# IanYeung/RealVSR

Hardware: AMD Instinct MI355X
Metric: HR frames/sec (fwd+bwd) on 5-frame 180x320 LR windows (higher is better)
Workload: dtype f32 (bf16x3 GEMM); 1 GPU; EDVR-M nf64, 5-frame 180x320 LR windows, batch 8 per GPU, x4 output, VideoSRModel.optimize_parameters: fwd + LapPyr(ssim,cb) on Y + GWLoss on CbCr + bwd + Adam step; per_gpu_batch=8, global_batch=8, parallelism=sequence-dp1, gemm=bf16x3 (3-term bf16 split on v_mfma_f32_32x32x16_bf16, f32 accumulate), lf_term=ssim (restated IQA_pytorch.SSIM, parity unpinned)

## Files before the change

### realvsr_amd/csrc/conv2_kernels.hip

```cpp
#define RVSR_DEFINE_PACK
#include "conv_plan.h"

#include "bf16x3.h"

#ifdef RVSR_ABL5
constexpr int ABL5 = RVSR_ABL5;
#else
constexpr int ABL5 = 0;
#endif

#ifdef RVSR_TIMELINE
__device__ unsigned long long rvsr_dbg[512];
extern "C" int rvsr_debug_read(unsigned long long* out) { return (int)hipMemcpyFromSymbol(out, HIP_SYMBOL(rvsr_dbg), sizeof(unsigned long long) * 512); }
#define STAMP(i) do { if (blockIdx.x == 77 && tid == 0) rvsr_dbg[(i)] = __builtin_amdgcn_s_memtime(); } while (0)
#else
#define STAMP(i) do {} while (0)
#endif

template <int MT, int MODE>
__device__ __forceinline__ void conv2_epilogue(f32x16 (&acc)[MT][2], const ConvFwdParams& p, const float* bias_s, int b,
                                               int o0, int row0, int col, int hi) {
    const float neg = p.act == 0 ? 1.f : (p.act == 1 ? 0.f : p.slope);
    const bool col_ok = col < p.Wout;
    const size_t HW = (size_t)p.Hout * p.Wout;
// ... 76 lines not shown
                float4 v = make_float4(r0 + bb, r1 + bb, r2 + bb, r3 + bb);
                v.x = v.x > 0.f ? v.x : v.x * neg; v.y = v.y > 0.f ? v.y : v.y * neg;
                v.z = v.z > 0.f ? v.z : v.z * neg; v.w = v.w > 0.f ? v.w : v.w * neg;
                if (MODE == 1) { v.x += resv[rg].x; v.y += resv[rg].y; v.z += resv[rg].z; v.w += resv[rg].w; }
                buf_store4(out_rs, off[rg] + (unsigned)(o0 + m * 32 + 8 * rg) * HW4, 0u, v);
            }
        }
    }
}

__device__ __forceinline__ void half_swap(float& a, float& b) {
    asm volatile("s_nop 1\n\tv_permlane32_swap_b32 %0, %1\n\ts_nop 0" : "+v"(a), "+v"(b));
}
template <int MT, int MODE>
__device__ __forceinline__ void conv2_epilogue_wide(f32x16 (&acc)[MT][2], const ConvFwdParams& p, const float* bias_s, int b,
                                                    int o0, int row, int x0, int lo, int hi) {
    if (row >= p.Hout) return;
    const float neg = (p.act == 0 || MODE == 4) ? 1.f : (p.act == 1 ? 0.f : p.slope);
    const int lane = 32 * hi + lo, jn = lane >> 4, Gn = lane & 15;
    const int src4 = 4 * (4 * Gn + jn);
    const int col4 = x0 + 4 * Gn;
    const bool col_ok = col4 < p.Wout;
    const unsigned HW = (unsigned)(p.Hout * p.Wout), HW4 = 4u * HW;
    const __amdgpu_buffer_rsrc_t out_rs = buf_view_2g(p.out1 + (size_t)b * p.Co * HW);
    const __amdgpu_buffer_rsrc_t res_rs = buf_view_2g(MODE == 5   ? p.res + (size_t)(b % p.res_period) * p.Co * HW
                                                      : MODE == 1 || MODE == 4 ? p.res + (size_t)b * p.Co * HW
                                                                               : p.out1);
    const unsigned lane_off = 4u * ((unsigned)jn * HW + (unsigned)row * p.Wout + col4);
    const int j = lo & 3;
#pragma unroll
    for (int m = 0; m < MT; ++m) {
#pragma unroll
        for (int rg = 0; rg < 4; ++rg) {
            float4 resv[2];
            unsigned off[2];
#pragma unroll
            for (int s = 0; s < 2; ++s) {
                const int ob = o0 + m * 32 + 8 * rg + 4 * s;
                off[s] = col_ok && ob + jn < p.Co ? lane_off : 0x80000000u;
                if (MODE == 1 || MODE == 4 || MODE == 5) {
                    typedef float f32x4v __attribute__((ext_vector_type(4)));
                    const f32x4v q = __builtin_bit_cast(f32x4v, __builtin_amdgcn_raw_buffer_load_b128(res_rs, (int)(off[s] + (unsigned)ob * HW4), 0, 0));
                    resv[s] = make_float4(q.x, q.y, q.z, q.w);
                }
            }
            float r[2][4];
            const float bb = bias_s[m * 32 + 8 * rg + 4 * hi + j];
#pragma unroll
            for (int n = 0; n < 2; ++n) {
                r[n][0] = acc[m][n][4 * rg + 0]; r[n][1] = acc[m][n][4 * rg + 1]; r[n][2] = acc[m][n][4 * rg + 2]; r[n][3] = acc[m][n][4 * rg + 3];
                quad_transpose4(r[n][0], r[n][1], r[n][2], r[n][3], lo);
#pragma unroll
                for (int e = 0; e < 4; ++e) {
                    const float v = r[n][e] + bb;
                    r[n][e] = MODE == 5 ? v : (v > 0.f ? v : v * neg);
                }
            }
#pragma unroll
            for (int e = 0; e < 4; ++e) half_swap(r[0][e], r[1][e]);
#pragma unroll
            for (int s = 0; s < 2; ++s)
#pragma unroll
                for (int e = 0; e < 4; ++e)
                    r[s][e] = __builtin_bit_cast(float, __builtin_amdgcn_ds_bpermute(src4, __builtin_bit_cast(int, r[s][e])));
#pragma unroll
            for (int s = 0; s < 2; ++s) {
                float4 v = make_float4(r[s][0], r[s][1], r[s][2], r[s][3]);
                if (MODE == 1 || MODE == 5) { v.x += resv[s].x; v.y += resv[s].y; v.z += resv[s].z; v.w += resv[s].w; }
                if (MODE == 5) {
                    v.x = v.x > 0.f ? v.x : v.x * neg; v.y = v.y > 0.f ? v.y : v.y * neg;
                    v.z = v.z > 0.f ? v.z : v.z * neg; v.w = v.w > 0.f ? v.w : v.w * neg;
                }
                if (MODE == 4) {
                    v.x *= resv[s].x > 0.f ? 1.f : p.slope; v.y *= resv[s].y > 0.f ? 1.f : p.slope;
                    v.z *= resv[s].z > 0.f ? 1.f : p.slope; v.w *= resv[s].w > 0.f ? 1.f : p.slope;
                }
                if (!(ABL5 & 2) || (m == 0 && rg == 0 && s == 0))
                buf_store4(out_rs, off[s] + (unsigned)(o0 + m * 32 + 8 * rg + 4 * s) * HW4, 0u, v);
            }
        }
    }
}

template <int KS, int STRIDE, int MT, int CCG, bool ACT_IN, int NW>
__global__ __launch_bounds__(NW * 64, 2) void conv_fwd2_kernel(const ConvFwdParams p) {
    constexpr int T = KS * KS, PAD = KS / 2, TH = 2 * NW, TW = 32, NTHR = NW * 64;
    constexpr int IH = (TH - 1) * STRIDE + KS, IW = (TW - 1) * STRIDE + KS;
    constexpr int MP = MT * 32, NOCT = 2 * CCG, NPOS = IH * IW;
    constexpr int WVEC = T * NOCT * MP;
    extern __shared__ __attribute__((aligned(16))) unsigned char smem_raw[];
    bf16x8* xs_hi = reinterpret_cast<bf16x8*>(smem_raw);
    bf16x8* xs_lo = xs_hi + NOCT * NPOS;
    bf16x8* ws_hi = xs_lo + NOCT * NPOS;
    bf16x8* ws_lo = ws_hi + WVEC;
    float* bias_s = reinterpret_cast<float*>(ws_lo + WVEC);
    const int tid = threadIdx.x, lane = tid & 63, wave = tid >> 6, lo = lane & 31, hi = lane >> 5;
    const TView& va = p.in.a;
    const TView& vb = p.in.b;
    const int C1 = va.C, Ctot = va.C + vb.C;
    const int nchunks = (Ctot + 16 * CCG - 1) / (16 * CCG);

    const unsigned nmb = (p.Co + MP - 1) / MP, nty = (p.Hout + TH - 1) / TH, ntx = (p.Wout + TW - 1) / TW;
    const unsigned items = ntx * nty * nmb * p.B;
    const unsigned xcd = blockIdx.x & 7, wq = blockIdx.x >> 3, nwq = (gridDim.x + 7 - xcd) >> 3;
    const unsigned q8 = items >> 3, r8 = items & 7;
    const unsigned range0 = xcd < r8 ? xcd * (q8 + 1) : r8 * (q8 + 1) + (xcd - r8) * q8;
    const unsigned range1 = range0 + q8 + (xcd < r8 ? 1 : 0);

    int x0 = 0, y0 = 0, mb = 0, b = 0;
    auto decode = [&](unsigned S) {
        const unsigned t = S % (p.ntx * nty);
        x0 = (int)(t % p.ntx) * TW;
        y0 = (int)(t / p.ntx) * TH;
        mb = (int)((S / (p.ntx * nty)) % nmb);
        b = (int)(S / (p.ntx * nty * nmb));
    };

    constexpr int NIT = (NOCT * NPOS + NTHR - 1) / NTHR;
    constexpr int NWV = (2 * WVEC + NTHR - 1) / NTHR;
    float vin[NIT][8];
    float ain[ACT_IN ? NIT : 1][8];
    int nvalid[NIT];

    __amdgpu_buffer_rsrc_t xa_rs = buf_view_2g(va.p), xb_rs = buf_view_2g(va.p), act_rs = buf_view_2g(va.p);
    auto tile_views = [&]() {
        if (va.mode != 0) return;
        const size_t hw = (size_t)va.Hs * va.Ws;
        xa_rs = buf_view_2g(va.p + (size_t)b * va.C * hw);
        if (vb.C) xb_rs = buf_view_2g(vb.p + (size_t)b * vb.C * hw);
        if (ACT_IN) act_rs = buf_view_2g(va.act + (size_t)b * va.C * hw);
    };
    auto issue_loads = [&](int chunk, int i_lo = 0, int i_hi = 1 << 20) {
        const int c0 = chunk * 16 * CCG;
#pragma unroll
        for (int i = 0; i < NIT; ++i) {
            if (i < i_lo || i >= i_hi) continue;
            const int it_raw = tid + i * NTHR;
            const bool live = it_raw < NOCT * NPOS;
            const int it = live ? it_raw : 0;
            const int oc = it / NPOS, pos = it - oc * NPOS;
            const int r = pos / IW, s = pos - r * IW;
            const int gy = y0 * STRIDE - PAD + r, gx = x0 * STRIDE - PAD + s;
            const int cb = c0 + oc * 8;
            const bool inb = live && gy >= 0 && gx >= 0 && gy < va.Hv && gx < va.Wv && cb < Ctot;
            const int gyc = gy < 0 ? 0 : (gy >= va.Hv ? va.Hv - 1 : gy), gxc = gx < 0 ? 0 : (gx >= va.Wv ? va.Wv - 1 : gx);
            if (va.mode == 0) {
                const bool second = c0 >= C1;
                const int Cb = second ? vb.C : va.C, cl0 = second ? c0 - C1 : c0;
                const unsigned hw4 = 4u * (unsigned)(va.Hs * va.Ws);
                const bool pos_ok = live && gy >= 0 && gx >= 0 && gy < va.Hv && gx < va.Wv;
                const unsigned vo = pos_ok ? 4u * (unsigned)(gy * va.Ws + gx) + (unsigned)(8 * oc) * hw4 : 0x80000000u;
                const int lane_nch = Cb - cl0 - 8 * oc;
                nvalid[i] = 8;
#pragma unroll
                for (int j = 0; j < 8; ++j) {
                    const unsigned vo_j = j < lane_nch ? vo : 0x80000000u;
                    const unsigned so = (unsigned)(cl0 + j) * hw4;
                    vin[i][j] = buf_load(second ? xb_rs : xa_rs, vo_j, so);
                    if (ACT_IN) ain[i][j] = buf_load(act_rs, vo_j, so);
                }
            } else {
                const size_t hw = (size_t)va.Hs * va.Ws;
                const int cbc = inb ? cb : 0;
                const size_t base = ((size_t)b * (va.C >> 2) + (cbc >> 2)) * hw + (size_t)(2 * gyc) * va.Ws + 2 * gxc;
                nvalid[i] = inb ? 8 : 0;
#pragma unroll
                for (int j = 0; j < 8; ++j) {
                    const size_t idx = base + (j >> 2) * hw + ((j >> 1) & 1) * va.Ws + (j & 1);
                    vin[i][j] = va.p[idx];
                    if (ACT_IN) ain[i][j] = va.act[idx];
                }
            }
        }
    };
    auto commit_inputs = [&](int i_lo = 0, int i_hi = 1 << 20) {
#pragma unroll
        for (int i = 0; i < NIT; ++i) {
            if (i < i_lo || i >= i_hi) continue;
            const int it = tid + i * NTHR;
            float v[8];
#pragma unroll
            for (int j = 0; j < 8; ++j) {
                float x = ACT_IN ? vin[i][j] * (ain[i][j] > 0.f ? 1.f : va.slope) : vin[i][j];
                v[j] = j < nvalid[i] ? x : 0.f;
            }
            bf16x8 h8, l8;
            split8(v, h8, l8);
            if (it < NOCT * NPOS) {
                xs_hi[it] = h8;
                xs_lo[it] = l8;
            }
        }
    };
    auto commit_to_lds = [&](int chunk, bool inputs_done = false) {
        const bf16x8* src = reinterpret_cast<const bf16x8*>(p.wpack) + ((size_t)mb * nchunks + chunk) * 2 * WVEC;
        constexpr int WB = MT >= 4 ? 3 : 9;
        constexpr bool OVERLAP = !ACT_IN && MT <= 2;
        if (!OVERLAP && !inputs_done) commit_inputs();
#pragma unroll
        for (int base = 0; base < NWV; base += WB) {
            bf16x8 wv[WB];
#pragma unroll
            for (int i = 0; i < WB; ++i) {
                const int e = tid + (base + i) * NTHR;
                wv[i] = src[(base + i < NWV && e < 2 * WVEC) ? e : 0];
            }
            if (OVERLAP && base == 0 && !inputs_done) commit_inputs();
#pragma unroll
            for (int i = 0; i < WB; ++i) {
                const int e = tid + (base + i) * NTHR;
                if (base + i < NWV && e < 2 * WVEC) ws_hi[e] = wv[i];
            }
        }
        if (chunk == 0 && tid < MP) {
            const int o = mb * MP + tid;
            bias_s[tid] = (p.bias != nullptr && o < p.Co) ? p.bias[o] : 0.f;
        }
    };

    constexpr bool PF = !ACT_IN && MT <= 2 && STRIDE == 1;
    unsigned S = range0 + wq;
    if (S < range1) {
        decode(S);
        tile_views();
        if (PF) issue_loads(0);
    }
    for (; S < range1; S += nwq) {
        f32x16 acc[MT][2];
#pragma unroll
        for (int m = 0; m < MT; ++m) {
            acc[m][0] = zero16();
            acc[m][1] = zero16();
        }
        const int cx0 = x0, cy0 = y0, cmb = mb, cb_ = b;
        STAMP(0);
        for (int chunk = 0; chunk < nchunks; ++chunk) {
            constexpr int NB = 3;
            if (!PF && STRIDE == 2) {
#pragma unroll
                for (int i0 = 0; i0 < NIT; i0 += NB) {
                    issue_loads(chunk, i0, i0 + NB);
                    commit_inputs(i0, i0 + NB);
                }
                commit_to_lds(chunk, true);
            } else {
                if (!PF) issue_loads(chunk);
                commit_to_lds(chunk);
            }
            STAMP(1 + chunk * 5);
            __syncthreads();
            STAMP(2 + chunk * 5);
            if (PF && chunk + 1 < nchunks) issue_loads(chunk + 1);
            STAMP(3 + chunk * 5);
#pragma unroll
            for (int tap = 0; tap < T; ++tap) {
                const int dy = tap / KS, dx = tap % KS;
#pragma unroll
                for (int g = 0; g < CCG; ++g) {
                    const int oc = 2 * g + hi;
                    bf16x8 ah[MT], al[MT], bh[2], bl[2];
#pragma unroll
                    for (int m = 0; m < MT; ++m) {
                        ah[m] = ws_hi[(tap * NOCT + oc) * MP + m * 32 + lo];
                        al[m] = ws_lo[(tap * NOCT + oc) * MP + m * 32 + lo];
                    }
#pragma unroll
                    for (int n = 0; n < 2; ++n) {
                        const int idx = (oc * IH + (wave * 2 + n) * STRIDE + dy) * IW + lo * STRIDE + dx;
                        bh[n] = xs_hi[idx];
                        bl[n] = xs_lo[idx];
                    }
#pragma unroll
                    for (int m = 0; m < MT; ++m)
#pragma unroll
                        for (int n = 0; n < 2; ++n) acc[m][n] = mfma_bf16(ah[m], bh[n], acc[m][n]);
#pragma unroll
                    for (int m = 0; m < MT; ++m)
#pragma unroll
                        for (int n = 0; n < 2; ++n) acc[m][n] = mfma_bf16(ah[m], bl[n], acc[m][n]);
#pragma unroll
                    for (int m = 0; m < MT; ++m)
#pragma unroll
                        for (int n = 0; n < 2; ++n) acc[m][n] = mfma_bf16(al[m], bh[n], acc[m][n]);
                }
            }
            STAMP(4 + chunk * 5);
            __syncthreads();
            STAMP(5 + chunk * 5);
        }
        if (p.ps)
            conv2_epilogue<MT, 3>(acc, p, bias_s, cb_, cmb * MP, cy0 + wave * 2, cx0 + lo, hi);
        else if (p.out2 != nullptr)
            conv2_epilogue<MT, 2>(acc, p, bias_s, cb_, cmb * MP, cy0 + wave * 2, cx0 + lo, hi);
        else if (p.res != nullptr) {
            if (p.vec4) conv2_epilogue_v4<MT, 1>(acc, p, bias_s, cb_, cmb * MP, cy0 + wave * 2, cx0, lo, hi);
            else conv2_epilogue<MT, 1>(acc, p, bias_s, cb_, cmb * MP, cy0 + wave * 2, cx0 + lo, hi);
        } else {
            if (p.vec4) conv2_epilogue_v4<MT, 0>(acc, p, bias_s, cb_, cmb * MP, cy0 + wave * 2, cx0, lo, hi);
            else conv2_epilogue<MT, 0>(acc, p, bias_s, cb_, cmb * MP, cy0 + wave * 2, cx0 + lo, hi);
        }
        STAMP(30);
        if (S + nwq < range1) {
            decode(S + nwq);
// ... 384 lines not shown
            for (int m = 0; m < MT; ++m)
#pragma unroll
                for (int n = 0; n < 2; ++n) acc[m][n] = mfma_bf16(ah[sl][m], bh[sl][n], acc[m][n]);
            if (NT >= 2) {
#pragma unroll
                for (int m = 0; m < MT; ++m)
#pragma unroll
                    for (int n = 0; n < 2; ++n) acc[m][n] = mfma_bf16(ah[sl][m], bl[sl][n], acc[m][n]);
            }
            if (NT >= 3) {
#pragma unroll
                for (int m = 0; m < MT; ++m)
#pragma unroll
                    for (int n = 0; n < 2; ++n) acc[m][n] = mfma_bf16(al[sl][m], bh[sl][n], acc[m][n]);
            }
            }
            if (tap < 4) {
                if (pub) commit(buf ^ 1, NWV, tap);
            } else {
                if (pub) commit(buf ^ 1, tap - 4, 8);
                if (tap == 4) stage_tile(q + 2, k_nx2, c_nx2);
                issue_stage(q + 2, c_nx2, tap - 4, (ABL5 & 4) ? 8 : VEC ? (tap < 6 ? tap - 4 : 8) : (tap - 4 < NIT ? tap - 4 : 8));
            }
            __builtin_amdgcn_sched_barrier(0);
        }
        STAMP(2 + (q & 7) * 3);
#ifdef RVSR_TIMELINE
        if (blockIdx.x == 77 && lane == 0 && q == Q - 3) rvsr_dbg[70 + wave] = __builtin_amdgcn_s_memtime();
        if (blockIdx.x == 77 && lane == 0 && q == Q - 4) rvsr_dbg[90 + wave] = __builtin_amdgcn_s_memtime();
        if (blockIdx.x == 77 && lane == 0 && q == Q - 6) rvsr_dbg[300 + wave * 12 + 9] = __builtin_amdgcn_s_memtime();
#endif
        const int k = k_cur;
        const bool last_chunk = c_cur == nchunks - 1;
        if (++c_cur == nchunks) { c_cur = 0; ++k_cur; }
        if (++c_nx2 == nchunks) { c_nx2 = 0; ++k_nx2; }
        if (last_chunk) {
            const Tile cur = tile_of(k);
            const float* bias_s = bias_base + (k & 3) * MP;
            if (WIDE) {
                if (p.act == 3) conv2_epilogue_wide<MT, 4>(acc, p, bias_s, cur.b, cur.mb * MP, cur.y0 + wave, cur.x0, lo, hi);
                else if (p.res_period > 0) conv2_epilogue_wide<MT, 5>(acc, p, bias_s, cur.b, cur.mb * MP, cur.y0 + wave, cur.x0, lo, hi);
                else if (p.res != nullptr) conv2_epilogue_wide<MT, 1>(acc, p, bias_s, cur.b, cur.mb * MP, cur.y0 + wave, cur.x0, lo, hi);
                else conv2_epilogue_wide<MT, 0>(acc, p, bias_s, cur.b, cur.mb * MP, cur.y0 + wave, cur.x0, lo, hi);
            } else if (p.ps)
                conv2_epilogue<MT, 3>(acc, p, bias_s, cur.b, cur.mb * MP, cur.y0 + wave * 2, cur.x0 + lo, hi);
            else if (p.out2 != nullptr)
                conv2_epilogue<MT, 2>(acc, p, bias_s, cur.b, cur.mb * MP, cur.y0 + wave * 2, cur.x0 + lo, hi);
            else if (p.res != nullptr) {
                if (p.vec4) conv2_epilogue_v4<MT, 1>(acc, p, bias_s, cur.b, cur.mb * MP, cur.y0 + wave * 2, cur.x0, lo, hi);
                else conv2_epilogue<MT, 1>(acc, p, bias_s, cur.b, cur.mb * MP, cur.y0 + wave * 2, cur.x0 + lo, hi);
            } else {
                if (p.vec4) conv2_epilogue_v4<MT, 0>(acc, p, bias_s, cur.b, cur.mb * MP, cur.y0 + wave * 2, cur.x0, lo, hi);
                else conv2_epilogue<MT, 0>(acc, p, bias_s, cur.b, cur.mb * MP, cur.y0 + wave * 2, cur.x0 + lo, hi);
            }
#pragma unroll
            for (int m = 0; m < MT; ++m) {
                acc[m][0] = zero16();
                acc[m][1] = zero16();
            }
        }
        __syncthreads();
        STAMP(3 + (q & 7) * 3);
#ifdef RVSR_TIMELINE
        if (blockIdx.x == 77 && lane == 0 && q == Q - 4) rvsr_dbg[80 + wave] = __builtin_amdgcn_s_memtime();
        if (blockIdx.x == 77 && lane == 0 && q == Q - 6) rvsr_dbg[300 + wave * 12 + 10] = __builtin_amdgcn_s_memtime();
        if (blockIdx.x == 77 && lane == 0 && q == Q - 7) rvsr_dbg[300 + wave * 12 + 11] = __builtin_amdgcn_s_memtime();
#endif
    }
    STAMP(61);
#ifdef RVSR_TIMELINE
    if (blockIdx.x == 77 && tid == 0) rvsr_dbg[62] = (unsigned long long)Q;
#endif
}


size_t rvsr_conv_fwd2_workspace_bytes(int ksize, int Co, int Ctot) {
    int mt, ccg, nchunks, nmb;
    conv_fwd2_geom(ksize, Co, Ctot, mt, ccg, nchunks, nmb);
    return (size_t)nmb * nchunks * 2 * (ksize * ksize) * (2 * ccg) * (mt * 32) * 16;
}

typedef void (*ConvFwdKernel)(const ConvFwdParams);

static ConvFwdKernel fwd2_kernel(int ksize, int stride, const ConvFwdPlan& q) {
#define ROW(KS, STRIDE, MT, CCG) \
    if (ksize == KS && stride == STRIDE && q.mt == MT) return q.act_in ? conv_fwd2_kernel<KS, STRIDE, MT, CCG, true, 4> : conv_fwd2_kernel<KS, STRIDE, MT, CCG, false, 4>
    ROW(3, 2, 1, 1);
    ROW(3, 2, 2, 1);
    ROW(5, 1, 1, 1);
    ROW(5, 2, 1, 1);
    ROW(1, 1, 1, 2);
    ROW(1, 1, 2, 2);
#undef ROW
    return nullptr;
}

static ConvFwdKernel fwd5_kernel(const ConvFwdPlan& q) {
#define ROW(MT, VEC, WIDE, NT) \
    if (q.mt == MT && q.vec == VEC && q.wide == WIDE && q.nt == NT) return q.act_in ? conv_fwd5_kernel<MT, true, VEC, WIDE, NT> : conv_fwd5_kernel<MT, false, VEC, WIDE, NT>
    ROW(2, 1, true, 3);
    ROW(2, 1, true, 2);
    ROW(2, 1, true, 1);
    ROW(2, 1, false, 3);
    ROW(2, 1, false, 2);
    ROW(2, 1, false, 1);
    ROW(2, 2, false, 3);
    ROW(2, 2, false, 2);
    ROW(2, 2, false, 1);
    ROW(2, 3, false, 3);
    ROW(2, 3, false, 2);
    ROW(2, 3, false, 1);
    ROW(2, 0, false, 3);
    ROW(1, 0, false, 3);
    ROW(1, 1, false, 3);
    ROW(1, 2, false, 3);
    ROW(1, 3, false, 3);
#undef ROW
    if (q.mt == 2 && q.vec == 1 && q.nt == 4 && !q.act_in) return q.wide ? conv_fwd5_kernel<2, false, 1, true, 4> : conv_fwd5_kernel<2, false, 1, false, 4>;
    return nullptr;
}

int rvsr_launch_conv_fwd2(ConvFwdParams p, const ConvFwdPlan& q, int ksize, int stride, void* workspace, size_t workspace_bytes, hipStream_t st) {
    const int Ctot = p.in.a.C + p.in.b.C, T = ksize * ksize;
    int mt, ccg, nchunks, nmb;
    conv_fwd2_geom(ksize, p.Co, Ctot, mt, ccg, nchunks, nmb);
    const size_t need = rvsr_conv_fwd2_workspace_bytes(ksize, p.Co, Ctot);
    if (!workspace || workspace_bytes < need) FAIL(RVSR_ERR_WORKSPACE, "conv2d: workspace %zu B < %zu B", workspace_bytes, need);
    const bool five = q.family == CONV_FWD5;
    const ConvFwdKernel k = five ? fwd5_kernel(q) : fwd2_kernel(ksize, stride, q);
    if (!k) FAIL(RVSR_ERR_LAUNCH, "conv2d: no %s instantiation for this plan", five ? "conv_fwd5" : "conv_fwd2");
    if (!p.prepacked) {
        const size_t total = (size_t)nmb * nchunks * T * (2 * ccg) * (mt * 32);
        hipLaunchKernelGGL(pack_weights_kernel, dim3((unsigned)((total + 255) / 256)), dim3(256), 0, st, p.w, (bf16x8*)workspace, p.Co,
                           Ctot, T, mt * 32, ccg, nchunks, nmb, p.w_mode | (p.fmt ? 0x100 : 0));
    }
    p.wpack = workspace;
    p.vec4 = q.vec4;
    return rvsr_conv_launch(five ? "conv_fwd5" : "conv_fwd2", k, dim3(q.gx), five ? 512 : 256, q.lds, st, p);
}

extern "C" size_t rvsr_conv2d_pack_weights(const float* weight, int C_in, int Co, int ksize, int w_mode, void* out, size_t out_bytes,
                                           long long* desc, void* stream) {
    int mt, ccg, nchunks, nmb;
    if (ksize != 1 && ksize != 3 && ksize != 5) return 0;
    conv_fwd2_geom(ksize, Co, C_in, mt, ccg, nchunks, nmb);
    const size_t need = rvsr_conv_fwd2_workspace_bytes(ksize, Co, C_in);
    if (!weight || !out || out_bytes < need) return 0;
    if ((w_mode & 4) && !conv_f16fp8_ok(ksize, 1, mt, w_mode & 1)) return 0;
    const int fmtflag = (w_mode & 4) ? 0x100 : 0;
    const int T = ksize * ksize;
    const size_t total = (size_t)nmb * nchunks * T * (2 * ccg) * (mt * 32);
    hipLaunchKernelGGL(pack_weights_kernel, dim3((unsigned)((total + 255) / 256)), dim3(256), 0, (hipStream_t)stream, weight, (bf16x8*)out, Co,
                       C_in, T, mt * 32, ccg, nchunks, nmb, (w_mode & 1) | fmtflag);
    if (desc) {
        desc[0] = (long long)(uintptr_t)weight; desc[1] = (long long)(uintptr_t)out;
        desc[2] = Co; desc[3] = C_in; desc[4] = T; desc[5] = mt * 32; desc[6] = ccg; desc[7] = nchunks; desc[8] = nmb; desc[9] = (w_mode & 1) | fmtflag;
    }
    return need;
}
extern "C" int rvsr_pack_weights_batched(const void* descs, int n, void* stream) {
    if (n <= 0) return RVSR_OK;
    if (!descs) FAIL(RVSR_ERR_BAD_ARG, "pack_weights_batched: null table");
    static_assert(sizeof(PackDesc) == 48, "PackDesc layout is part of the C ABI (two pointers + eight ints)");
    hipLaunchKernelGGL(pack_weights_batched_kernel, dim3(16, (unsigned)n), dim3(256), 0, (hipStream_t)stream, (const PackDesc*)descs);
    hipError_t e = hipGetLastError();
    if (e != hipSuccess) FAIL(RVSR_ERR_LAUNCH, "pack_weights_batched launch: %s", hipGetErrorString(e));
    return RVSR_OK;
}

#define WG2_THREADS 512
#define WG2_GP 272
#define WG2_XP 496

typedef unsigned int u32x4 __attribute__((ext_vector_type(4)));

__device__ __forceinline__ bf16x8 as_bf16x8(u32x4 v) { return __builtin_bit_cast(bf16x8, v); }

template <int SHIFT>
__device__ __forceinline__ bf16x8 take8(u32x4 a, u32x4 b) {
    u32x4 r;
    if (SHIFT == 4) {
        r[0] = a[2]; r[1] = a[3]; r[2] = b[0]; r[3] = b[1];
    } else if (SHIFT == 3) {
        r[0] = __builtin_amdgcn_alignbit(a[2], a[1], 16);
        r[1] = __builtin_amdgcn_alignbit(a[3], a[2], 16);
        r[2] = __builtin_amdgcn_alignbit(b[0], a[3], 16);
        r[3] = __builtin_amdgcn_alignbit(b[1], b[0], 16);
    } else {
        r[0] = __builtin_amdgcn_alignbit(a[3], a[2], 16);
        r[1] = __builtin_amdgcn_alignbit(b[0], a[3], 16);
        r[2] = __builtin_amdgcn_alignbit(b[1], b[0], 16);
        r[3] = __builtin_amdgcn_alignbit(b[2], b[1], 16);
    }
    return as_bf16x8(r);
}

template <int DXMASK, int NT>
__device__ __forceinline__ void wg2_row(const unsigned char* xs_hi, const unsigned char* xs_lo, int xoff, bf16x8 ah,
                                        bf16x8 al, f32x16* acc) {
    const u32x4 h0 = *reinterpret_cast<const u32x4*>(xs_hi + xoff), h1 = *reinterpret_cast<const u32x4*>(xs_hi + xoff + 16);
    constexpr int N = ((DXMASK >> 0) & 1) + ((DXMASK >> 1) & 1) + ((DXMASK >> 2) & 1);
    bf16x8 bh[3], bl[3];
    int t = 0;
    if (DXMASK & 1) { bh[t] = take8<3>(h0, h1); ++t; }
    if (DXMASK & 2) { bh[t] = take8<4>(h0, h1); ++t; }
    if (DXMASK & 4) { bh[t] = take8<5>(h0, h1); ++t; }
    if (NT >= 2) {
        const u32x4 l0 = *reinterpret_cast<const u32x4*>(xs_lo + xoff), l1 = *reinterpret_cast<const u32x4*>(xs_lo + xoff + 16);
        t = 0;
        if (DXMASK & 1) { bl[t] = take8<3>(l0, l1); ++t; }
        if (DXMASK & 2) { bl[t] = take8<4>(l0, l1); ++t; }
        if (DXMASK & 4) { bl[t] = take8<5>(l0, l1); ++t; }
// ... 455 lines not shown
        }
    };
    auto commit = [&]() {
        {
            float v[8] = {gv[0].x, gv[0].y, gv[0].z, gv[0].w, gv[1].x, gv[1].y, gv[1].z, gv[1].w};
            if (ACT) {
                const float s[8] = {sv[0].x, sv[0].y, sv[0].z, sv[0].w, sv[1].x, sv[1].y, sv[1].z, sv[1].w};
#pragma unroll
                for (int j = 0; j < 8; ++j) v[j] *= s[j] > 0.f ? 1.f : p.g.slope;
            }
            bacc += ((v[0] + v[1]) + (v[2] + v[3])) + ((v[4] + v[5]) + (v[6] + v[7]));
            bf16x8 h8, l8;
            split8(v, h8, l8);
            *reinterpret_cast<bf16x8*>(t_hi + r64 * WG1_RP + q * 16) = h8;
            *reinterpret_cast<bf16x8*>(t_lo + r64 * WG1_RP + q * 16) = l8;
        }
#pragma unroll
        for (int i = 0; i < NXI; ++i) {
            if (i >= nblk) continue;
            const float v[8] = {xv[i][0].x, xv[i][0].y, xv[i][0].z, xv[i][0].w, xv[i][1].x, xv[i][1].y, xv[i][1].z, xv[i][1].w};
            bf16x8 h8, l8;
            split8(v, h8, l8);
            const int dst = (64 + 64 * i + r64) * WG1_RP + q * 16;
            *reinterpret_cast<bf16x8*>(t_hi + dst) = h8;
            *reinterpret_cast<bf16x8*>(t_lo + dst) = l8;
        }
    };

    f32x16 acc[3];
#pragma unroll
    for (int j = 0; j < 3; ++j) acc[j] = zero16();
    if (t_begin < t_end) issue_loads(t_begin, -1);
    for (int tile = t_begin; tile < t_end; ++tile) {
        const int next = tile + 1 < t_end ? tile + 1 : tile;
        commit();
        __syncthreads();
#pragma unroll
        for (int ks = 0; ks < WG1_KT / 16; ++ks) {
            issue_loads(next, ks);
            __builtin_amdgcn_sched_barrier(0);
            if (!m_live) continue;
            const int koff = ks * 32 + hi * 16;
            const int goff = (m * 32 + lo) * WG1_RP + koff;
            const bf16x8 ah = *reinterpret_cast<const bf16x8*>(t_hi + goff), al = *reinterpret_cast<const bf16x8*>(t_lo + goff);
#pragma unroll
            for (int j = 0; j < 3; ++j) {
                const int nt = ng + 4 * j;
                if (nt >= ntile) continue;
                const int xoff = (64 + nt * 32 + lo) * WG1_RP + koff;
                const bf16x8 bh = *reinterpret_cast<const bf16x8*>(t_hi + xoff), bl = *reinterpret_cast<const bf16x8*>(t_lo + xoff);
                acc[j] = mfma_bf16(ah, bh, acc[j]);
                acc[j] = mfma_bf16(ah, bl, acc[j]);
                acc[j] = mfma_bf16(al, bh, acc[j]);
            }
        }
        __syncthreads();
    }

    float* part = p.part + (size_t)blockIdx.x * p.Co * Ctot;
#pragma unroll
    for (int j = 0; j < 3; ++j) {
        const int nt = ng + 4 * j, c = c0 + nt * 32 + lo;
        if (!m_live || nt >= ntile || c >= Ctot) continue;
#pragma unroll
        for (int r = 0; r < 16; ++r) {
            const int o = o0 + m * 32 + drow(r, hi);
            if (o < p.Co) part[(size_t)o * Ctot + c] = acc[j][r];
        }
    }
    if (do_bias) {
        float v = bacc;
        v += __shfl_xor(v, 1);
        v += __shfl_xor(v, 2);
        v += __shfl_xor(v, 4);
        if (q == 0 && o0 + r64 < p.Co) p.bpart[(size_t)blockIdx.x * p.Co + o0 + r64] = v;
    }
}

int rvsr_launch_conv_wgrad1x1s(const ConvWgradParams& p, int gy, int gz, hipStream_t st) {
    auto k = p.g.act != nullptr ? conv_wgrad1x1s_kernel<true> : conv_wgrad1x1s_kernel<false>;
    return rvsr_conv_launch("conv_wgrad1x1s", k, dim3(p.P, gy, gz), WG1_THREADS, (size_t)2 * WG1_ROWS * WG1_RP, st, p);
}

template <bool ACT>
__global__ __launch_bounds__(256, 2) void conv_wgrad_s2_kernel(const ConvWgradParams p) {
    const int tid = threadIdx.x, lane = tid & 63, wave = tid >> 6, lo = lane & 31, hi = lane >> 5;
    const int m = wave & 1, n = wave >> 1;
    const int C = p.x.a.C;
    const int Hin = p.x.a.Hs, Win = p.x.a.Ws;
    const int Ho = p.Hout, Wo = p.Wout;
    const int o = blockIdx.y * 64 + m * 32 + lo;
    const int c = blockIdx.z * 64 + n * 32 + lo;
    const bool o_ok = o < p.Co, c_ok = c < C;
    const int oc = o_ok ? o : 0, cc = c_ok ? c : 0;
    const int UW = (Wo + 15) / 16;
    const long units = (long)p.B * Ho * UW;
    const long per = (units + p.P - 1) / p.P;
    long u0 = (long)blockIdx.x * per, u1 = u0 + per;
    if (u1 > units) u1 = units;
    f32x16 acc[9];
#pragma unroll
    for (int t = 0; t < 9; ++t) acc[t] = zero16();
    float bsum = 0.f;
    for (long u = u0; u < u1; ++u) {
        const int b = (int)(u / ((long)Ho * UW));
        const int rem = (int)(u - (long)b * Ho * UW);
        const int py = rem / UW, px0 = (rem - py * UW) * 16 + 8 * hi;
        const bool pv = px0 < Wo;
        const size_t gidx = (((size_t)b * p.Co + oc) * Ho + py) * Wo + (pv ? px0 : 0);
        const float4 g0 = *reinterpret_cast<const float4*>(p.g.p + gidx), g1 = *reinterpret_cast<const float4*>(p.g.p + gidx + 4);
        float4 a0, a1;
        if (ACT) {
            a0 = *reinterpret_cast<const float4*>(p.g.act + gidx);
            a1 = *reinterpret_cast<const float4*>(p.g.act + gidx + 4);
        }
        float xr[3][20];
#pragma unroll
        for (int dy = 0; dy < 3; ++dy) {
            const int iy = 2 * py + dy - 1;
            const bool rok = pv && c_ok && iy >= 0 && iy < Hin;
            const float* row = p.x.a.p + (((size_t)b * C + cc) * Hin + (rok ? iy : 0)) * Win;
#pragma unroll
            for (int j = 0; j < 5; ++j) {
                const int col = 2 * px0 - 4 + 4 * j;
                const bool ok = rok && col >= 0 && col < Win;
                const float4 q = *reinterpret_cast<const float4*>(row + (ok ? col : 0));
                xr[dy][4 * j + 0] = ok ? q.x : 0.f; xr[dy][4 * j + 1] = ok ? q.y : 0.f;
                xr[dy][4 * j + 2] = ok ? q.z : 0.f; xr[dy][4 * j + 3] = ok ? q.w : 0.f;
            }
        }
        float gv[8] = {g0.x, g0.y, g0.z, g0.w, g1.x, g1.y, g1.z, g1.w};
        if (ACT) {
            const float av[8] = {a0.x, a0.y, a0.z, a0.w, a1.x, a1.y, a1.z, a1.w};
#pragma unroll
            for (int j = 0; j < 8; ++j) gv[j] *= av[j] > 0.f ? 1.f : p.g.slope;
        }
        const bool gok = pv && o_ok;
#pragma unroll
        for (int j = 0; j < 8; ++j) {
            gv[j] = gok ? gv[j] : 0.f;
            bsum += gv[j];
        }
        bf16x8 gh, gl;
        split8(gv, gh, gl);
#pragma unroll
        for (int dy = 0; dy < 3; ++dy) {
#pragma unroll
            for (int dx = 0; dx < 3; ++dx) {
                float xv[8];
#pragma unroll
                for (int i = 0; i < 8; ++i) xv[i] = xr[dy][3 + dx + 2 * i];
                bf16x8 xh, xl;
                split8(xv, xh, xl);
                f32x16& a = acc[dy * 3 + dx];
                a = mfma_bf16(gh, xh, a);
                a = mfma_bf16(gh, xl, a);
                a = mfma_bf16(gl, xh, a);
            }
        }
    }
    float* part = p.part + (size_t)blockIdx.x * p.Co * C * 9;
#pragma unroll
    for (int t = 0; t < 9; ++t) {
#pragma unroll
        for (int r = 0; r < 16; ++r) {
            const int orow = blockIdx.y * 64 + m * 32 + drow(r, hi);
            if (orow < p.Co && c_ok) part[((size_t)orow * C + c) * 9 + t] = acc[t][r];
        }
    }
    if (p.bpart != nullptr && blockIdx.z == 0 && n == 0) {
        bsum += __shfl_xor(bsum, 32);
        if (hi == 0 && o_ok) p.bpart[(size_t)blockIdx.x * p.Co + o] = bsum;
    }
}

int rvsr_launch_conv_wgrad_s2(const ConvWgradParams& p, int gy, int gz, hipStream_t st) {
    auto k = p.g.act != nullptr ? conv_wgrad_s2_kernel<true> : conv_wgrad_s2_kernel<false>;
    return rvsr_conv_launch("conv_wgrad_s2", k, dim3(p.P, gy, gz), 256, 0, st, p);
}

template <int STRIDE, int NT>
__global__ __launch_bounds__(256, 1) void conv_wgrad5_kernel(const ConvWgradParams p) {
    constexpr int KS = 5, T = 25, PAD = 2, TH = 4, TW = 32, NPX = TH * TW, TPW = 7;
    constexpr int IH = (TH - 1) * STRIDE + KS, IW = (TW - 1) * STRIDE + KS;
    constexpr int CS = (IH * IW) | 1, GS = NPX + 1;
    extern __shared__ __attribute__((aligned(16))) float smem5[];
    float* gT = smem5;
    float* xs = smem5 + 32 * GS;
    const int tid = threadIdx.x, lane = tid & 63, wave = tid >> 6, lo = lane & 31, hi = lane >> 5;
    const int mb = blockIdx.y, c0 = blockIdx.z * 32;
    const int Ctot = p.x.a.C + p.x.b.C;
    int xoff[TPW];
#pragma unroll
    for (int i = 0; i < TPW; ++i) {
        const int tap = wave + 4 * i;
        xoff[i] = tap < T ? lo * CS + (tap / KS) * IW + (tap % KS) : 0;
    }
    f32x16 acc[TPW];
#pragma unroll
    for (int i = 0; i < TPW; ++i) {
        acc[i] = zero16();
        asm volatile("" : "+v"(acc[i]));
    }
    float bsum = 0.f;
    const int ntiles = p.B * p.nty * p.ntx;
    for (int tile = blockIdx.x; tile < ntiles; tile += p.P) {
        const int b = tile / (p.nty * p.ntx);
        const int trem = tile - b * (p.nty * p.ntx);
        const int ty = trem / p.ntx, tx = trem - ty * p.ntx;
        const int y0 = ty * TH, x0 = tx * TW;
#pragma unroll 4
        for (int e = tid; e < 32 * NPX; e += 256) {
            const int ol = e / NPX, px = e - ol * NPX;
            gT[ol * GS + px] = tview_get(p.g, b, mb * 32 + ol, y0 + (px >> 5), x0 + (px & 31));
        }
#pragma unroll 4
        for (int e = tid; e < 32 * IH * IW; e += 256) {
            const int cc = e / (IH * IW), rem = e - cc * (IH * IW);
            const int r = rem / IW, s = rem - r * IW;
            xs[cc * CS + r * IW + s] = tcat_get(p.x, b, c0 + cc, y0 * STRIDE - PAD + r, x0 * STRIDE - PAD + s);
        }
        __syncthreads();
        if (p.bpart != nullptr && blockIdx.z == 0 && tid < 32) {
            float s = 0.f;
            for (int px = 0; px < NPX; ++px) s += gT[tid * GS + px];
            bsum += s;
        }
#pragma unroll 1
        for (int ks = 0; ks < NPX / 16; ++ks) {
            const int row = ks >> 1, col0 = (ks & 1) * 16 + 8 * hi;
            float av[8];
#pragma unroll
            for (int q = 0; q < 8; ++q) av[q] = gT[lo * GS + row * 32 + col0 + q];
            bf16x8 ah, al;
            split8(av, ah, al);
            const int poff = row * STRIDE * IW + col0 * STRIDE;
#pragma unroll
            for (int i = 0; i < TPW; ++i) {
                if (wave + 4 * i >= T) continue;
                float bv[8];
#pragma unroll
                for (int q = 0; q < 8; ++q) bv[q] = xs[xoff[i] + poff + q * STRIDE];
                bf16x8 bh, bl;
                split8(bv, bh, bl);
                acc[i] = mfma_bf16(ah, bh, acc[i]);
                if (NT >= 2) acc[i] = mfma_bf16(ah, bl, acc[i]);
                if (NT >= 3) acc[i] = mfma_bf16(al, bh, acc[i]);
            }
        }
        __syncthreads();
    }
#pragma unroll
    for (int i = 0; i < TPW; ++i) {
        const int tap = wave + 4 * i, c = c0 + lo;
        if (tap >= T || c >= Ctot) continue;
#pragma unroll
        for (int r = 0; r < 16; ++r) {
            const int o = mb * 32 + drow(r, hi);
            if (o < p.Co) p.part[(((size_t)blockIdx.x * p.Co + o) * Ctot + c) * T + tap] = acc[i][r];
        }
    }
// ... 23 lines not shown
```

### realvsr_amd/csrc/conv_plan.h

```cpp
#pragma once
#include "conv_common.h"

static inline bool conv_al16(const void* a, const void* b = nullptr, const void* c = nullptr, const void* d = nullptr) {
    return ((((uintptr_t)a) | ((uintptr_t)b) | ((uintptr_t)c) | ((uintptr_t)d)) & 15) == 0;
}
static inline bool conv_span_ok(size_t H, size_t W, size_t C) { return sizeof(float) * H * W * C < ((size_t)1 << 31); }


enum ConvFwdFamily {
    CONV_FWD_THIN = 0,
    CONV_FWD5 = 1,
    CONV_FWD2 = 2,
    CONV_FWD_F32 = 3,
};

struct ConvFwdPlan {
    int rc;
    const char* msg;
    int family;
    int mt;
    int vec;
    int wide;
    int nt;
    int act_in;
    int cc;
    int vec4;
    int th, tw;
    unsigned gx, gy, gz;
    size_t lds;
};

static inline void conv_fwd2_geom(int ksize, int Co, int Ctot, int& mt, int& ccg, int& nchunks, int& nmb) {
    mt = (Co <= 32 || ksize == 5) ? 1 : 2;
    ccg = ksize == 1 ? 2 : 1;
    nchunks = (Ctot + 16 * ccg - 1) / (16 * ccg);
    nmb = (Co + mt * 32 - 1) / (mt * 32);
}
static inline bool conv_f16fp8_ok(int ksize, int stride, int mt, int w_mode) { return ksize == 3 && stride == 1 && mt == 2 && w_mode == 0; }

#define THIN_FW 136
#define THIN_FPL (10 * THIN_FW)
static inline bool conv_fwd_thin_ok(const ConvFwdParams& p, int ksize, int stride) {
    const TView& va = p.in.a;
    return ksize == 3 && stride == 1 && p.Co <= 4 && p.in.b.C == 0 && va.C % 8 == 0 && va.mode == 0 && va.act == nullptr &&
           p.out2 == nullptr && !p.ps && p.w_mode == 0 && p.Wout % 4 == 0 && va.Ws == p.Wout && va.Hs == p.Hout &&
           conv_al16(va.p, p.out1, p.res) && conv_span_ok(p.Hout, p.Wout, va.C) && va.C <= 256;
}

static inline ConvFwdPlan conv_fwd_refusal(const char* msg) {
    ConvFwdPlan r = {};
    r.rc = RVSR_ERR_UNSUPPORTED;
    r.msg = msg;
    r.family = -1;
    return r;
}

static inline ConvFwdPlan conv_fwd_plan(const ConvFwdParams& p, int ksize, int stride, int gemm_mode) {
    const TView& va = p.in.a;
    const TView& vb = p.in.b;
    const int Ctot = va.C + vb.C, T = ksize * ksize;
    if (p.act == 3 && (!p.res || ksize != 3 || stride != 1 || p.ps || p.out2 || gemm_mode == 1)) return conv_fwd_refusal(nullptr);
    if (p.res_period > 0 && (p.act == 3 || ksize != 3 || stride != 1 || p.ps || p.out2 || gemm_mode == 1)) return conv_fwd_refusal(nullptr);
    ConvFwdPlan q = {};
    q.act_in = va.act != nullptr;
    q.nt = 3;
    q.th = 8;
    q.tw = 32;
    int ccg, nchunks, nmb;
    conv_fwd2_geom(ksize, p.Co, Ctot, q.mt, ccg, nchunks, nmb);
    const int ntx = (p.Wout + 31) / 32, nty8 = (p.Hout + 7) / 8;

    bool split = p.act == 3 || p.res_period > 0;
    const bool thin = !split && conv_fwd_thin_ok(p, ksize, stride);
    if (!split && !thin) {
        split = gemm_mode != 1 && (va.mode != 1 || ksize == 3) && (vb.C == 0 || va.C % 8 == 0);
        if (split && (ksize != 3 || stride == 2) && va.mode == 0 &&
            (!conv_span_ok(va.Hs, va.Ws, va.C > vb.C ? va.C : vb.C) || (vb.C != 0 && va.C % (16 * ccg) != 0)))
            split = false;
    }
    if (p.fmt && !(split && conv_f16fp8_ok(ksize, stride, q.mt, p.w_mode)))
        return conv_fwd_refusal("conv2d: the f16 + fp8 format (w_mode | 4) is for forward 3x3 / stride-1 convs with more than 32 output channels");

    if (thin) {
        q.family = CONV_FWD_THIN;
        q.mt = 1;
        q.tw = 128;
        q.gx = (unsigned)p.B * nty8 * ((p.Wout + 127) / 128);
        q.gy = q.gz = 1;
        q.lds = sizeof(float) * (8 * THIN_FPL + (size_t)va.C * 36);
        return q;
    }
    if (!split) {
        q.family = CONV_FWD_F32;
        q.mt = p.Co <= 32 ? 1 : (p.Co <= 64 ? 2 : 4);
        const int wide_m = q.mt == 4;
        q.cc = ksize == 1 ? 32 : ksize == 3 ? (stride == 1 ? (wide_m ? 8 : 16) : (wide_m ? 4 : 8)) : (stride == 1 ? (wide_m ? 4 : 8) : 4);
        const int IH = 7 * stride + ksize, IW = 31 * stride + ksize;
        q.lds = sizeof(float) * ((size_t)q.cc * IH * IW + (size_t)T * q.cc * (q.mt * 32 + 1));
        q.gx = (unsigned)(ntx * nty8);
        q.gy = (unsigned)((p.Co + q.mt * 32 - 1) / (q.mt * 32));
        q.gz = (unsigned)p.B;
        return q;
    }
    q.vec4 = (p.Wout % 4 == 0) && conv_al16(p.out1, p.res) && !p.ps && p.out2 == nullptr && conv_span_ok(p.Hout, p.Wout, p.Co);
    q.cc = ccg;
    q.gy = q.gz = 1;
    long items = (long)nmb * p.B;
    if (ksize != 3 || stride != 1) {
        q.family = CONV_FWD2;
        const int IH = 7 * stride + ksize, IW = 31 * stride + ksize;
        q.lds = (size_t)16 * (2 * (2 * ccg) * IH * IW + 2 * T * (2 * ccg) * (q.mt * 32)) + sizeof(float) * q.mt * 32;
        items *= (long)ntx * nty8;
        const int slots = 256 * (q.lds > 80 * 1024 ? 1 : 2);
        q.gx = (unsigned)(items < slots ? items : slots);
        return q;
    }
    q.family = CONV_FWD5;
    const bool al = conv_al16(va.p, va.act, vb.p);
    if (va.mode == 0 && va.Ws % 4 == 0 && va.Wv == va.Ws && al && conv_span_ok(va.Hs, va.Ws, va.C > vb.C ? va.C : vb.C) &&
// ... 127 lines not shown
```

Measured before the change: 84.66 HR frames/s.

## Vectorize stride-2 conv staging, reorder tile decode, double-buffer stride-2 wgrad in LDS

Measured after the change: 85.12 HR frames/s, median of 6. Within noise of the previous version (+0.5%).

```diff
diff --git a/realvsr_amd/csrc/conv2_kernels.hip b/realvsr_amd/csrc/conv2_kernels.hip
--- a/realvsr_amd/csrc/conv2_kernels.hip
+++ b/realvsr_amd/csrc/conv2_kernels.hip
@@ -182,8 +182,9 @@
     }
 }
 
-template <int KS, int STRIDE, int MT, int CCG, bool ACT_IN, int NW>
-__global__ __launch_bounds__(NW * 64, 2) void conv_fwd2_kernel(const ConvFwdParams p) {
+template <int KS, int STRIDE, int MT, int CCG, bool ACT_IN, int NW, bool V16 = false>
+__global__ __launch_bounds__(NW * 64, V16 ? 1 : 2) void conv_fwd2_kernel(const ConvFwdParams p) {
+    static_assert(!V16 || (KS == 3 && STRIDE == 2 && !ACT_IN), "16-byte staging: the 3x3 / stride-2 forward instantiations only");
     constexpr int T = KS * KS, PAD = KS / 2, TH = 2 * NW, TW = 32, NTHR = NW * 64;
     constexpr int IH = (TH - 1) * STRIDE + KS, IW = (TW - 1) * STRIDE + KS;
     constexpr int MP = MT * 32, NOCT = 2 * CCG, NPOS = IH * IW;
@@ -209,18 +210,24 @@
 
     int x0 = 0, y0 = 0, mb = 0, b = 0;
     auto decode = [&](unsigned S) {
-        const unsigned t = S % (p.ntx * nty);
+        const unsigned t = (S / nmb) % (p.ntx * nty);
         x0 = (int)(t % p.ntx) * TW;
         y0 = (int)(t / p.ntx) * TH;
-        mb = (int)((S / (p.ntx * nty)) % nmb);
+        mb = (int)(S % nmb);
         b = (int)(S / (p.ntx * nty * nmb));
     };
 
     constexpr int NIT = (NOCT * NPOS + NTHR - 1) / NTHR;
     constexpr int NWV = (2 * WVEC + NTHR - 1) / NTHR;
+    constexpr bool PF = V16 || (MT <= 2 && STRIDE == 1 && (!ACT_IN || KS == 1));
+    constexpr bool PF_ACT = PF && ACT_IN;
     float vin[NIT][8];
     float ain[ACT_IN ? NIT : 1][8];
     int nvalid[NIT];
+    typedef float f32x4v __attribute__((ext_vector_type(4)));
+    constexpr int NG = (IW + 6) / 4, NIT4 = V16 ? (NOCT * IH * NG + NTHR - 1) / NTHR : 1;
+    f32x4v vq[NIT4][8];
+    bf16x8 wpre[V16 ? NWV : 1];
 
     __amdgpu_buffer_rsrc_t xa_rs = buf_view_2g(va.p), xb_rs = buf_view_2g(va.p), act_rs = buf_view_2g(va.p);
     auto tile_views = [&]() {
@@ -230,12 +237,68 @@
         if (vb.C) xb_rs = buf_view_2g(vb.p + (size_t)b * vb.C * hw);
         if (ACT_IN) act_rs = buf_view_2g(va.act + (size_t)b * va.C * hw);
     };
+    auto issue_loads_v = [&](int chunk) {
+        const int c0 = chunk * 16 * CCG;
+        const bool second = c0 >= C1;
+        const int Cb = second ? vb.C : va.C, cl0 = second ? c0 - C1 : c0;
+        const unsigned hw4 = 4u * (unsigned)(va.Hs * va.Ws);
+        const __amdgpu_buffer_rsrc_t rs = second ? xb_rs : xa_rs;
+#pragma unroll
+        for (int i = 0; i < NIT4; ++i) {
+            const int it_raw = tid + i * NTHR;
+            const bool live = it_raw < NOCT * IH * NG;
+            const int it = live ? it_raw : 0;
+            const int oc = it / (IH * NG), rem = it - oc * (IH * NG);
+            const int r = rem / NG, g = rem - r * NG;
+            const int gy = y0 * STRIDE - PAD + r, col = x0 * STRIDE - 4 + 4 * g;
+            const bool pos_ok = live && gy >= 0 && gy < va.Hv && col >= 0 && col < va.Ws;
+            const unsigned vo = pos_ok ? 4u * (unsigned)(gy * va.Ws + col) + (unsigned)(8 * oc) * hw4 : 0x80000000u;
+            const int lane_nch = Cb - cl0 - 8 * oc;
+#pragma unroll
+            for (int j = 0; j < 8; ++j)
+                vq[i][j] = __builtin_bit_cast(f32x4v, __builtin_amdgcn_raw_buffer_load_b128(rs, (int)(j < lane_nch ? vo : 0x80000000u),
+                                                                                            (int)((unsigned)(cl0 + j) * hw4), 0));
+        }
+        const bf16x8* src = reinterpret_cast<const bf16x8*>(p.wpack) + ((size_t)mb * nchunks + chunk) * 2 * WVEC;
+#pragma unroll
+        for (int i = 0; i < NWV; ++i) {
+            const int e = tid + i * NTHR;
+            wpre[i] = src[e < 2 * WVEC ? e : 0];
+        }
+    };
+    auto commit_inputs_v = [&]() {
+#pragma unroll
+        for (int i = 0; i < NIT4; ++i) {
+            const int it = tid + i * NTHR;
+            const int oc = it / (IH * NG), rem = it - oc * (IH * NG);
+            const int r = rem / NG, g = rem - r * NG;
+#pragma unroll
+            for (int e = 0; e < 4; ++e) {
+                const int s = 4 * g - 3 + e;
+                float v[8];
+#pragma unroll
+                for (int j = 0; j < 8; ++j) v[j] = vq[i][j][e];
+                bf16x8 h8, l8;
+                split8(v, h8, l8);
+                if (it < NOCT * IH * NG && s >= 0 && s < IW) {
+                    xs_hi[(oc * IH + r) * IW + s] = h8;
+                    xs_lo[(oc * IH + r) * IW + s] = l8;
+                }
+            }
+        }
+    };
     auto issue_loads = [&](int chunk, int i_lo = 0, int i_hi = 1 << 20) {
+        if constexpr (V16) {
+            issue_loads_v(chunk);
+            return;
+        }
         const int c0 = chunk * 16 * CCG;
+        int t = tid;
+        if constexpr (PF_ACT) asm volatile("" : "+v"(t));
 #pragma unroll
         for (int i = 0; i < NIT; ++i) {
             if (i < i_lo || i >= i_hi) continue;
-            const int it_raw = tid + i * NTHR;
+            const int it_raw = t + i * NTHR;
             const bool live = it_raw < NOCT * NPOS;
             const int it = live ? it_raw : 0;
             const int oc = it / NPOS, pos = it - oc * NPOS;
@@ -274,6 +337,10 @@
         }
     };
     auto commit_inputs = [&](int i_lo = 0, int i_hi = 1 << 20) {
+        if constexpr (V16) {
+            commit_inputs_v();
+            return;
+        }
 #pragma unroll
         for (int i = 0; i < NIT; ++i) {
             if (i < i_lo || i >= i_hi) continue;
@@ -293,6 +360,19 @@
         }
     };
     auto commit_to_lds = [&](int chunk, bool inputs_done = false) {
+        if constexpr (V16) {
+            commit_inputs();
+#pragma unroll
+            for (int i = 0; i < NWV; ++i) {
+                const int e = tid + i * NTHR;
+                if (e < 2 * WVEC) ws_hi[e] = wpre[i];
+            }
+            if (chunk == 0 && tid < MP) {
+                const int o = mb * MP + tid;
+                bias_s[tid] = (p.bias != nullptr && o < p.Co) ? p.bias[o] : 0.f;
+            }
+            return;
+        }
         const bf16x8* src = reinterpret_cast<const bf16x8*>(p.wpack) + ((size_t)mb * nchunks + chunk) * 2 * WVEC;
         constexpr int WB = MT >= 4 ? 3 : 9;
         constexpr bool OVERLAP = !ACT_IN && MT <= 2;
@@ -318,7 +398,6 @@
         }
     };
 
-    constexpr bool PF = !ACT_IN && MT <= 2 && STRIDE == 1;
     unsigned S = range0 + wq;
     if (S < range1) {
         decode(S);
@@ -869,7 +948,8 @@
 
 typedef void (*ConvFwdKernel)(const ConvFwdParams);
 
-static ConvFwdKernel fwd2_kernel(int ksize, int stride, const ConvFwdPlan& q) {
+static ConvFwdKernel fwd2_kernel(int ksize, int stride, const ConvFwdPlan& q, bool v16) {
+    if (v16 && ksize == 3 && stride == 2 && !q.act_in) return q.mt == 1 ? conv_fwd2_kernel<3, 2, 1, 1, false, 4, true> : conv_fwd2_kernel<3, 2, 2, 1, false, 4, true>;
 #define ROW(KS, STRIDE, MT, CCG) \
     if (ksize == KS && stride == STRIDE && q.mt == MT) return q.act_in ? conv_fwd2_kernel<KS, STRIDE, MT, CCG, true, 4> : conv_fwd2_kernel<KS, STRIDE, MT, CCG, false, 4>
     ROW(3, 2, 1, 1);
@@ -914,7 +994,7 @@
     const size_t need = rvsr_conv_fwd2_workspace_bytes(ksize, p.Co, Ctot);
     if (!workspace || workspace_bytes < need) FAIL(RVSR_ERR_WORKSPACE, "conv2d: workspace %zu B < %zu B", workspace_bytes, need);
     const bool five = q.family == CONV_FWD5;
-    const ConvFwdKernel k = five ? fwd5_kernel(q) : fwd2_kernel(ksize, stride, q);
+    const ConvFwdKernel k = five ? fwd5_kernel(q) : fwd2_kernel(ksize, stride, q, conv_fwd2_vec_staging(p, ksize, stride));
     if (!k) FAIL(RVSR_ERR_LAUNCH, "conv2d: no %s instantiation for this plan", five ? "conv_fwd5" : "conv_fwd2");
     if (!p.prepacked) {
         const size_t total = (size_t)nmb * nchunks * T * (2 * ccg) * (mt * 32);
@@ -1536,8 +1616,15 @@
     return rvsr_conv_launch("conv_wgrad1x1s", k, dim3(p.P, gy, gz), WG1_THREADS, (size_t)2 * WG1_ROWS * WG1_RP, st, p);
 }
 
+constexpr int WS2_XRS = 36, WS2_GRS = 20;
+constexpr int WS2_XF = 64 * 3 * WS2_XRS, WS2_BUF = WS2_XF + 64 * WS2_GRS;
+constexpr int WS2_NX = 64 * 3 * 9, WS2_NI = (WS2_NX + 255) / 256;
+constexpr size_t WS2_LDS = sizeof(float) * (2 * WS2_BUF + WS2_XRS);
 template <bool ACT>
 __global__ __launch_bounds__(256, 2) void conv_wgrad_s2_kernel(const ConvWgradParams p) {
+    extern __shared__ __attribute__((aligned(16))) unsigned char smem_raw[];
+    float* sm = reinterpret_cast<float*>(smem_raw);
+    float* zrow = sm + 2 * WS2_BUF;
     const int tid = threadIdx.x, lane = tid & 63, wave = tid >> 6, lo = lane & 31, hi = lane >> 5;
     const int m = wave & 1, n = wave >> 1;
     const int C = p.x.a.C;
@@ -1546,7 +1633,6 @@
     const int o = blockIdx.y * 64 + m * 32 + lo;
     const int c = blockIdx.z * 64 + n * 32 + lo;
     const bool o_ok = o < p.Co, c_ok = c < C;
-    const int oc = o_ok ? o : 0, cc = c_ok ? c : 0;
     const int UW = (Wo + 15) / 16;
     const long units = (long)p.B * Ho * UW;
     const long per = (units + p.P - 1) / p.P;
@@ -1556,54 +1642,85 @@
 #pragma unroll
     for (int t = 0; t < 9; ++t) acc[t] = zero16();
     float bsum = 0.f;
-    for (long u = u0; u < u1; ++u) {
+
+    const int sg_row = tid >> 2, sg_q = tid & 3;
+    const int sg_o = blockIdx.y * 64 + sg_row;
+    const bool sg_ok = sg_o < p.Co;
+    float4 gq = make_float4(0.f, 0.f, 0.f, 0.f), aq = gq, xq[WS2_NI];
+    unsigned xok = 0;
+    bool gok = false;
+    auto load_unit = [&](long u) {
         const int b = (int)(u / ((long)Ho * UW));
         const int rem = (int)(u - (long)b * Ho * UW);
-        const int py = rem / UW, px0 = (rem - py * UW) * 16 + 8 * hi;
-        const bool pv = px0 < Wo;
-        const size_t gidx = (((size_t)b * p.Co + oc) * Ho + py) * Wo + (pv ? px0 : 0);
-        const float4 g0 = *reinterpret_cast<const float4*>(p.g.p + gidx), g1 = *reinterpret_cast<const float4*>(p.g.p + gidx + 4);
-        float4 a0, a1;
+        const int py = rem / UW, ux = rem - py * UW;
+        gok = sg_ok && ux * 16 + 4 * sg_q < Wo;
+        const size_t gidx = (((size_t)b * p.Co + (sg_ok ? sg_o : 0)) * Ho + py) * Wo + (gok ? ux * 16 + 4 * sg_q : 0);
+        gq = *reinterpret_cast<const float4*>(p.g.p + gidx);
+        if (ACT) aq = *reinterpret_cast<const float4*>(p.g.act + gidx);
+        xok = 0;
+        int t = tid;
+        asm volatile("" : "+v"(t));
+#pragma unroll
+        for (int i = 0; i < WS2_NI; ++i) {
+            const int e_raw = t + 256 * i;
+            const int e = e_raw < WS2_NX ? e_raw : 0;
+            const int xr_ = e / 27, r27 = e - xr_ * 27, dy = r27 / 9, j = r27 - dy * 9;
+            const int xc = blockIdx.z * 64 + xr_;
+            const int iy = 2 * py + dy - 1, col = 32 * ux - 4 + 4 * j;
+            const bool ok = xc < C && iy >= 0 && iy < Hin && col >= 0 && col < Win;
+            xok |= ok ? 1u << i : 0u;
+            xq[i] = *reinterpret_cast<const float4*>(p.x.a.p + (((size_t)b * C + (xc < C ? xc : 0)) * Hin + (ok ? iy : 0)) * Win + (ok ? col : 0));
+        }
+    };
+    auto store_unit = [&](int k) {
+        float* buf = sm + k * WS2_BUF;
+        float4 g = gq;
         if (ACT) {
-            a0 = *reinterpret_cast<const float4*>(p.g.act + gidx);
-            a1 = *reinterpret_cast<const float4*>(p.g.act + gidx + 4);
-        }
-        float xr[3][20];
-#pragma unroll
-        for (int dy = 0; dy < 3; ++dy) {
-            const int iy = 2 * py + dy - 1;
-            const bool rok = pv && c_ok && iy >= 0 && iy < Hin;
-            const float* row = p.x.a.p + (((size_t)b * C + cc) * Hin + (rok ? iy : 0)) * Win;
-#pragma unroll
-            for (int j = 0; j < 5; ++j) {
-                const int col = 2 * px0 - 4 + 4 * j;
-                const bool ok = rok && col >= 0 && col < Win;
-                const float4 q = *reinterpret_cast<const float4*>(row + (ok ? col : 0));
-                xr[dy][4 * j + 0] = ok ? q.x : 0.f; xr[dy][4 * j + 1] = ok ? q.y : 0.f;
-                xr[dy][4 * j + 2] = ok ? q.z : 0.f; xr[dy][4 * j + 3] = ok ? q.w : 0.f;
-            }
-        }
-        float gv[8] = {g0.x, g0.y, g0.z, g0.w, g1.x, g1.y, g1.z, g1.w};
-        if (ACT) {
-            const float av[8] = {a0.x, a0.y, a0.z, a0.w, a1.x, a1.y, a1.z, a1.w};
-#pragma unroll
-            for (int j = 0; j < 8; ++j) gv[j] *= av[j] > 0.f ? 1.f : p.g.slope;
-        }
-        const bool gok = pv && o_ok;
-#pragma unroll
-        for (int j = 0; j < 8; ++j) {
-            gv[j] = gok ? gv[j] : 0.f;
-            bsum += gv[j];
-        }
+            g.x *= aq.x > 0.f ? 1.f : p.g.slope; g.y *= aq.y > 0.f ? 1.f : p.g.slope;
+            g.z *= aq.z > 0.f ? 1.f : p.g.slope; g.w *= aq.w > 0.f ? 1.f : p.g.slope;
+        }
+        if (!gok) g = make_float4(0.f, 0.f, 0.f, 0.f);
+        *reinterpret_cast<float4*>(buf + WS2_XF + sg_row * WS2_GRS + 4 * sg_q) = g;
+#pragma unroll
+        for (int i = 0; i < WS2_NI; ++i) {
+            const int e = tid + 256 * i;
+            const float4 q = (xok >> i) & 1u ? xq[i] : make_float4(0.f, 0.f, 0.f, 0.f);
+            if (e < WS2_NX) *reinterpret_cast<float4*>(buf + 4 * e) = q;
+        }
+    };
+    if (tid < WS2_XRS) zrow[tid] = 0.f;
+    if (u0 < u1) {
+        load_unit(u0);
+        store_unit(0);
+    }
+    __syncthreads();
+    int k = 0;
+    for (long u = u0; u < u1; ++u, k ^= 1) {
+        load_unit(u + 1 < u1 ? u + 1 : u);
+        const int ux = (int)(u % UW);
+        const bool pv = ux * 16 + 8 * hi < Wo;
+        const float* buf = sm + k * WS2_BUF;
+        const float* gp = buf + WS2_XF + (m * 32 + lo) * WS2_GRS + 8 * hi;
+        const float4 g0 = *reinterpret_cast<const float4*>(gp), g1 = *reinterpret_cast<const float4*>(gp + 4);
+        const float gv[8] = {g0.x, g0.y, g0.z, g0.w, g1.x, g1.y, g1.z, g1.w};
+#pragma unroll
+        for (int j = 0; j < 8; ++j) bsum += gv[j];
         bf16x8 gh, gl;
         split8(gv, gh, gl);
 #pragma unroll
         for (int dy = 0; dy < 3; ++dy) {
+            const float* xp = pv ? buf + ((n * 32 + lo) * 3 + dy) * WS2_XRS + 16 * hi : zrow;
+            float xr[20];
+#pragma unroll
+            for (int j = 0; j < 5; ++j) {
+                const float4 q = *reinterpret_cast<const float4*>(xp + 4 * j);
+                xr[4 * j + 0] = q.x; xr[4 * j + 1] = q.y; xr[4 * j + 2] = q.z; xr[4 * j + 3] = q.w;
+            }
 #pragma unroll
             for (int dx = 0; dx < 3; ++dx) {
                 float xv[8];
 #pragma unroll
-                for (int i = 0; i < 8; ++i) xv[i] = xr[dy][3 + dx + 2 * i];
+                for (int i = 0; i < 8; ++i) xv[i] = xr[3 + dx + 2 * i];
                 bf16x8 xh, xl;
                 split8(xv, xh, xl);
                 f32x16& a = acc[dy * 3 + dx];
@@ -1612,6 +1729,8 @@
                 a = mfma_bf16(gl, xh, a);
             }
         }
+        store_unit(k ^ 1);
+        __syncthreads();
     }
     float* part = p.part + (size_t)blockIdx.x * p.Co * C * 9;
 #pragma unroll
@@ -1630,7 +1749,7 @@
 
 int rvsr_launch_conv_wgrad_s2(const ConvWgradParams& p, int gy, int gz, hipStream_t st) {
     auto k = p.g.act != nullptr ? conv_wgrad_s2_kernel<true> : conv_wgrad_s2_kernel<false>;
-    return rvsr_conv_launch("conv_wgrad_s2", k, dim3(p.P, gy, gz), 256, 0, st, p);
+    return rvsr_conv_launch("conv_wgrad_s2", k, dim3(p.P, gy, gz), 256, WS2_LDS, st, p);
 }
 
 template <int STRIDE, int NT>
diff --git a/realvsr_amd/csrc/conv_plan.h b/realvsr_amd/csrc/conv_plan.h
--- a/realvsr_amd/csrc/conv_plan.h
+++ b/realvsr_amd/csrc/conv_plan.h
@@ -35,6 +35,10 @@
     ccg = ksize == 1 ? 2 : 1;
     nchunks = (Ctot + 16 * ccg - 1) / (16 * ccg);
     nmb = (Co + mt * 32 - 1) / (mt * 32);
+}
+static inline bool conv_fwd2_vec_staging(const ConvFwdParams& p, int ksize, int stride) {
+    const TView& va = p.in.a;
+    return ksize == 3 && stride == 2 && va.act == nullptr && va.mode == 0 && va.Ws % 4 == 0 && va.Wv == va.Ws && conv_al16(va.p, p.in.b.p);
 }
 static inline bool conv_f16fp8_ok(int ksize, int stride, int mt, int w_mode) { return ksize == 3 && stride == 1 && mt == 2 && w_mode == 0; }
 
```
